# ethz-asl/object_keypoints

Hardware: AMD Instinct MI355X
Metric: frames/sec keypoint inference (511x511 -> heatmaps+3D) (higher is better)
Workload: dtype bf16

## Files before the change

### object_keypoints_amd/csrc/okp_fire2.hip

```cpp
#include <cstdio>
#include <cstring>

#include <cstdlib>

#include "okp_internal.h"

#ifdef OKP_F2_ABL_NOSTORE
#define F2_STORE(v, rs, off) do { if ((off) == 0x7ffffff0u) __builtin_amdgcn_raw_buffer_store_b128(v, rs, (int)(off), 0, 0); } while (0)
#else
#define F2_STORE(v, rs, off) __builtin_amdgcn_raw_buffer_store_b128(v, rs, (int)(off), 0, 0)
#endif


namespace {

constexpr uint32_t kInvalid = 0x80000000u;
typedef __attribute__((address_space(3))) void* lds_ptr_t;
typedef float f32x2 __attribute__((ext_vector_type(2)));

constexpr int SP = 128;
constexpr int PBI = 6;
constexpr int NST = 4;
constexpr int MAXIH = 6;
#ifndef OKP_F2_DIH
#define OKP_F2_DIH 5
#endif
constexpr int kDwmIH = OKP_F2_DIH;
static_assert(kDwmIH >= 1 && kDwmIH <= 5, "DWM tile: (rows + 2) x 18 squeeze pixels <= SP");
#ifdef OKP_F2_NO_REMAP
constexpr int XST = SP * 64;
#else
constexpr int XST = SP * 64 + 64;
#endif

template <int MID> struct FireLds {
  static constexpr int OFF_S = 0;
  static constexpr int OFF_X = OFF_S + SP * MID * 2;
  static constexpr int OFF_WD = OFF_X + NST * XST;
  static constexpr int OFF_TAB = OFF_WD + 10 * MID * 4;
  static constexpr int OFF_MASK = OFF_TAB + 2 * 96 * 4;
  static constexpr int BYTES = OFF_MASK + 16;
};

template <typename T>
__device__ __forceinline__ u32x4 relu_add_pack8(const f32x4& a0, const f32x4& a1, const u32x4& r) {
  u32x4 v;
#pragma unroll
  for (int b = 0; b < 2; ++b) {
    const f32x4& a = b ? a1 : a0;
#pragma unroll
    for (int h = 0; h < 2; ++h) {
      const f32x2 s2 = f32x2{a[2 * h], a[2 * h + 1]} + f32x2{H16<T>::lo(r[2 * b + h]), H16<T>::hi(r[2 * b + h])};
      v[2 * b + h] = okp_pack2<T>(s2[0], s2[1]);
    }
  }
  typedef short s16x8 __attribute__((ext_vector_type(8)));
  const s16x8 z = {0, 0, 0, 0, 0, 0, 0, 0};
  return __builtin_bit_cast(u32x4, __builtin_elementwise_max(__builtin_bit_cast(s16x8, v), z));
}

__device__ __forceinline__ int fastdiv(int x, const OkpFastDiv& f) {
  return f.mul ? (int)(__umulhi((uint32_t)x, f.mul) >> f.shift) : x;
}

__device__ __forceinline__ void wait_vm(int n) {
  switch (n) {
    case 0: asm volatile("s_waitcnt vmcnt(0)" ::: "memory"); break;
    case 1: asm volatile("s_waitcnt vmcnt(1)" ::: "memory"); break;
    case 2: asm volatile("s_waitcnt vmcnt(2)" ::: "memory"); break;
    case 3: asm volatile("s_waitcnt vmcnt(3)" ::: "memory"); break;
    case 4: asm volatile("s_waitcnt vmcnt(4)" ::: "memory"); break;
    case 5: asm volatile("s_waitcnt vmcnt(5)" ::: "memory"); break;
    case 6: asm volatile("s_waitcnt vmcnt(6)" ::: "memory"); break;
    case 7: asm volatile("s_waitcnt vmcnt(7)" ::: "memory"); break;
    default: asm volatile("s_waitcnt vmcnt(8)" ::: "memory"); break;
  }
}

#ifdef OKP_FIRE_STAMPS
#define F2_STAMP_ANY(i) do { if (lane == 0 && blockIdx.x < 16) { uint64_t t_; asm volatile("s_memtime %0\n s_waitcnt lgkmcnt(0)" : "=s"(t_) :: "memory"); p.dbg[(blockIdx.x * 8 + w) * 8 + (i)] = (uint32_t)t_; } } while (0)
#define F2_STAMP(i) do { if (second && lane == 0 && blockIdx.x < 16) { uint64_t t_; asm volatile("s_memtime %0\n s_waitcnt lgkmcnt(0)" : "=s"(t_) :: "memory"); p.dbg[(blockIdx.x * 8 + w) * 8 + (i)] = (uint32_t)t_; } } while (0)
#else
#define F2_STAMP(i) do {} while (0)
#define F2_STAMP_ANY(i) do {} while (0)
#endif

template <typename T, int CIN, int MID, int STR, bool DWM = false>
__global__ __launch_bounds__(MID * 2, MID == 128 ? 2 : 1) void okp_fire2_kernel(const OkpFire2Params p) {
  static_assert(STR == 1 || STR == 2, "stride of both branches");
  constexpr bool DWM2 = DWM && STR == 2;
  constexpr int D2H = 3, D2W = 8, D2SW = 2 * (D2W - 1) + 3, D2SH = 2 * (D2H - 1) + 3, D2B = 2;
  static_assert(D2SH * D2SW <= SP && D2B * 16 >= D2H * D2W + 8, "stride-2 matrix-pipe tile");
  constexpr int DIH = kDwmIH;
  constexpr int DSW = 18;
  constexpr int NSB = !DWM ? SP / 16 : STR == 1 ? ((DIH + 2) * DSW + 15) / 16 : (D2SH * D2SW + 15) / 16;
  constexpr int NW = MID / 32;
  constexpr int NT = 64 * NW;
  constexpr int HALF = MID;
  constexpr int KS1 = CIN / 32;
  constexpr int KS2 = MID / 32;
#ifdef OKP_F2_RESIDENT_W1
  constexpr bool RES = CIN <= 256;
  constexpr int DWB = 1;
#else
  constexpr bool RES = false;
#ifdef OKP_F2_RESIDENT_WA
  constexpr int DWB = (CIN == 256 && MID == 128) ? OKP_F2_RESIDENT_WA : 1;
#else
  constexpr int DWB = (CIN == 256 && MID == 128) ? 4 : 1;
#endif
#endif
#ifndef OKP_F2_RESWA
#define OKP_F2_RESWA 0
#endif
#ifdef OKP_F2_RESIDENT_WA
  constexpr bool RESWA = CIN == 256 && MID == 128;
#else
  constexpr bool RESWA = OKP_F2_RESWA && DWM && CIN == 256 && MID == 128;
#endif
  constexpr bool WRING = !RES && MID >= 192;
#ifndef OKP_F2_PIPE
#define OKP_F2_PIPE 0
#endif
  constexpr bool PIPE = OKP_F2_PIPE && DWM && CIN == 256 && MID == 128 && !RES && !WRING;
  constexpr int NWS = PIPE ? 4 : 3;
  constexpr int DW = !WRING ? 0 : MID == 192 ? 5 : 3;
  constexpr int SWM = ((MID / 8) % 16 == 0) ? 15 : 7;
  constexpr int CG = MID / 8;
  constexpr int NDM = (SP / 16 + NW - 1) / NW;
  constexpr bool RING_SKIP = STR == 1 && CIN == 2 * MID && KS1 / 2 <= NST;
  using L = FireLds<MID>;
  constexpr int OFF_S = L::OFF_S, OFF_X = L::OFF_X, OFF_WD = L::OFF_WD, OFF_TAB = L::OFF_TAB, OFF_MASK = L::OFF_MASK;
  constexpr int OFF_W1 = (L::BYTES + 1023) / 1024 * 1024;
  constexpr int LDS_TOTAL = WRING ? OFF_W1 + DW * NW * 2048 : L::BYTES;
  static_assert(NT / CG == 16 && LDS_TOTAL <= 160 * 1024, "thread mapping / LDS");
  __shared__ __attribute__((aligned(16))) char smem[LDS_TOTAL];
  const int tid = threadIdx.x;
  const int lane = tid & 63;
  const int w = __builtin_amdgcn_readfirstlane(tid >> 6);
  const int l16 = lane & 15, q = lane >> 4;

  const __amdgpu_buffer_rsrc_t rs_x = __builtin_amdgcn_make_buffer_rsrc(const_cast<void*>(p.x), 0, (int)p.x_bytes, 0x00020000);
  const __amdgpu_buffer_rsrc_t rs_o = __builtin_amdgcn_make_buffer_rsrc(p.out, 0, (int)p.out_bytes, 0x00020000);

  const int chq = 32 * w + 8 * q;
  const __amdgpu_buffer_rsrc_t rs_w1 = __builtin_amdgcn_make_buffer_rsrc(const_cast<void*>(p.w1), 0, NW * 2 * KS1 * 1024, 0x00020000);
  const uint32_t w1_voff = (uint32_t)lane * 16u;
  auto load_w1 = [&](int ks, u32x4 (&dst)[2]) {
#ifdef OKP_F2_ABL_NOWEIGHTS
    if (ks != 0) { dst[0] = u32x4{0x3c003c00u, 0u, 0u, 0u}; dst[1] = dst[0]; return; }
#endif
#pragma unroll
    for (int b = 0; b < 2; ++b)
      dst[b] = __builtin_amdgcn_raw_buffer_load_b128(rs_w1, (int)w1_voff, (int)(((uint32_t)(w * 2 + b) * KS1 + (uint32_t)ks) * 1024u), 0);
  };
  auto issue_w = [&](int ks) {
    if constexpr (WRING) {
#pragma unroll
      for (int b = 0; b < 2; ++b)
        __builtin_amdgcn_raw_ptr_buffer_load_lds(rs_w1, (lds_ptr_t)(smem + OFF_W1 + ((ks % DW) * NW + w) * 2048 + b * 1024), 16,
                                                 (int)(((uint32_t)(w * 2 + b) * KS1 + (uint32_t)ks) * 1024u + (uint32_t)lane * 16u), 0, 0, 0);
    }
  };
  auto first_weights = [&](u32x4 (&f)[RES ? KS1 : NWS][2]) {
    if constexpr (WRING) {
#pragma unroll
      for (int ks = 0; ks < DW; ++ks) issue_w(ks);
    } else if constexpr (!RES) {
      load_w1(0, f[0]); load_w1(1, f[1]);
    }
  };
  u32x4 w1f[RES ? KS1 : NWS][2];
  if constexpr (RES) {
#pragma unroll
    for (int ks = 0; ks < KS1; ++ks) load_w1(ks, w1f[ks]);
  }
  const u32x4* const wa_lane = static_cast<const u32x4*>(p.wa) + (size_t)w * 2 * KS2 * 64 + lane;
  u32x4 waf[2][KS2];
  if constexpr (RESWA) {
#pragma unroll
    for (int b = 0; b < 2; ++b)
#pragma unroll
      for (int ks = 0; ks < KS2; ++ks) waf[b][ks] = wa_lane[(size_t)(b * KS2 + ks) * 64];
  }
  const f32x4 b1v0 = *reinterpret_cast<const f32x4*>(p.b1 + chq), b1v1 = *reinterpret_cast<const f32x4*>(p.b1 + chq + 4);
  const f32x4 bav0 = *reinterpret_cast<const f32x4*>(p.ba + chq), bav1 = *reinterpret_cast<const f32x4*>(p.ba + chq + 4);
  uint32_t a_row[PBI], a_key[PBI];
#pragma unroll
  for (int pb = 0; pb < PBI; ++pb) {
    int ip = 16 * pb + l16;
    if (ip >= p.IP) ip = 0;
    const int iy = fastdiv(ip, p.div_iw), ix = ip - iy * p.IW;
    const int sp = (STR * iy + 1) * p.SW + STR * ix + 1;
    a_row[pb] = (uint32_t)sp * (MID * 2);
    a_key[pb] = (uint32_t)(sp & SWM);
  }
  const uint32_t xfrag_off = (uint32_t)l16 * 64u + (uint32_t)((q + 2 * (l16 >> 2)) & 3) * 16u;
  const uint32_t s_dst = (uint32_t)(OFF_S + l16 * (MID * 2) + (((4 * w + q) ^ (l16 & SWM)) << 4));
  constexpr bool UNI = (SP / 16) % NW == 0;
  const int nd = UNI ? NDM : (SP / 16 - w + NW - 1) / NW;
  int d_sy[NDM], d_sx[NDM];
  uint32_t d_chunk[NDM];
#pragma unroll
  for (int i = 0; i < NDM; ++i) {
    const int row = 16 * (w + NW * i) + (lane >> 2);
    d_sy[i] = fastdiv(row, p.div_sw);
    d_sx[i] = row - d_sy[i] * p.SW;
    if (row >= p.SH * p.SW) d_sy[i] = 1 << 20;
    d_chunk[i] = (uint32_t)(((lane & 3) - 2 * (row >> 2)) & 3) * 16u;
  }
  const int m_sy = tid < p.SH * p.SW ? fastdiv(tid, p.div_sw) : (1 << 20);
  const int m_sx = tid - fastdiv(tid, p.div_sw) * p.SW;

  auto tile_origin = [&](int slot, int& n, int& y0, int& x0) {
    const int xq = p.n_tiles >> 3, xr = p.n_tiles & 7, xcd = slot & 7;
    const int tile = (xcd < xr ? xcd * (xq + 1) : xr * (xq + 1) + (xcd - xr) * xq) + (slot >> 3);
    n = fastdiv(tile, p.div_tiles_frame);
    const int trem = tile - n * p.tiles_y * p.tiles_x;
    const int ty = fastdiv(trem, p.div_tiles_x);
    y0 = ty * p.IH;
    x0 = (trem - ty * p.tiles_x) * p.IW;
  };
  uint32_t d_off[NDM];
  auto tile_setup = [&](int tile) {
    int n, y0, x0;
    tile_origin(tile, n, y0, x0);
#pragma unroll
    for (int i = 0; i < NDM; ++i) {
      const int y = STR * y0 - 1 + d_sy[i], x = STR * x0 - 1 + d_sx[i];
// ... 535 lines not shown
          }
          } else {
#pragma unroll
          for (int sr = 0; sr < STR * (MAXIH - 1) + 3; ++sr) {
            if (sr < STR * (p.IH - 1) + 3) {
              const int sp = sr * p.SW + STR * ixc + dx;
              const u32x4 sv = *reinterpret_cast<const u32x4*>(smem + OFF_S + sp * (MID * 2) + ((cg ^ (sp & SWM)) << 4));
              f32x2 s2[4];
#pragma unroll
              for (int e = 0; e < 4; ++e) s2[e] = f32x2{H16<T>::lo(sv[e]), H16<T>::hi(sv[e])};
#pragma unroll
              for (int dy = 0; dy < 3; ++dy) {
                const int iy = (sr - dy) / STR;
                if (sr - dy >= 0 && (sr - dy) % STR == 0 && iy < MAXIH) {
#pragma unroll
                  for (int e = 0; e < 4; ++e) v[iy][e] = __builtin_elementwise_fma(s2[e], wt[dy][e], v[iy][e]);
                }
              }
            }
          }
          }
        }
#pragma unroll
        for (int iy = 0; iy < MAXIH; ++iy) {
          u32x4 o;
#pragma unroll
          for (int e = 0; e < 4; ++e) {
            const float lo = fmaxf(v[iy][e][0] + H16<T>::lo(rr[iy][e]), 0.f);
            const float hi = fmaxf(v[iy][e][1] + H16<T>::hi(rr[iy][e]), 0.f);
            o[e] = okp_pack2<T>(lo, hi);
          }
          F2_STORE(o, rs_o, oo[iy]);
        }
      }
    }
    F2_STAMP(4);
  }
  F2_STAMP_ANY(7);
}

}


bool okp_fire2_supported(int cin, int mid, int half, int stride) {
  if (half != mid) return false;
  if (stride == 1)
    return (cin == 256 && mid == 128) || (cin == 384 && mid == 192) || (cin == 512 && mid == 256) ||
           (cin == 384 && mid == 128) || (cin == 512 && mid == 192);
  return stride == 2 && ((cin == 256 && mid == 128) || (cin == 384 && mid == 192) || (cin == 384 && mid == 256) || (cin == 256 && mid == 192));
}

template <typename T>
static int launch_fire2_t(OkpFire2Params p, int cin, int mid, int stride, hipStream_t stream) {
  const long resident_wg = 256 * (mid == 128 ? 2 : 1);
  long best = -1;
  for (int ih = 1; ih <= p.Ho && ih <= MAXIH; ++ih)
    for (int iw = 1; iw <= p.Wo && iw <= 96; ++iw) {
      const int sh = stride * (ih - 1) + 3, sw = stride * (iw - 1) + 3;
      if (sh * sw > SP || ih * iw > 16 * PBI) continue;
      const long ty = (p.Ho + ih - 1) / ih, tx = (p.Wo + iw - 1) / iw;
      const long rounds = ((long)p.N * ty * tx + resident_wg - 1) / resident_wg;
      const long score = (rounds << 40) + (rounds == 1 ? (long)sh * sw + 8 * (16 - (iw < 16 ? iw : 16)) : ty * tx) * 4096 - iw;
      if (best < 0 || score < best) { best = score; p.IH = ih; p.IW = iw; p.SH = sh; p.SW = sw; p.tiles_y = (int)ty; p.tiles_x = (int)tx; }
    }
  if (stride == 2) {
    static const char* const e = getenv("OKP_F2_S2_TILE");
    int ih = 0, iw = 0;
    if (e && sscanf(e, "%d,%d", &ih, &iw) == 2 && ih >= 1 && ih <= MAXIH && iw >= 1 && (2 * (ih - 1) + 3) * (2 * (iw - 1) + 3) <= SP && ih * iw <= 16 * PBI) {
      p.IH = ih < p.Ho ? ih : p.Ho; p.IW = iw < p.Wo ? iw : p.Wo; p.SH = 2 * (p.IH - 1) + 3; p.SW = 2 * (p.IW - 1) + 3;
      p.tiles_y = (p.Ho + p.IH - 1) / p.IH; p.tiles_x = (p.Wo + p.IW - 1) / p.IW;
    }
  }
  static const bool dwm_on = [] { const char* e = getenv("OKP_F2_DWM"); return !(e && e[0] == '0'); }();
  static const int dwm_mid = [] { const char* e = getenv("OKP_F2_DWM_MID"); return e ? atoi(e) : 256; }();
  const bool dwm = dwm_on && stride == 1 && p.Wo % 16 == 0 && mid <= dwm_mid;
  if (dwm) {
    p.IH = p.Ho < kDwmIH ? p.Ho : kDwmIH; p.IW = 16; p.SH = p.IH + 2; p.SW = 18;
    p.tiles_y = (p.Ho + p.IH - 1) / p.IH; p.tiles_x = p.Wo / 16;
  }
  static const bool dwm2_on = [] { const char* e = getenv("OKP_F2_DWM_S2"); return !(e && e[0] == '0'); }();
  const bool dwm2 = dwm_on && dwm2_on && stride == 2 && p.Wo % 8 == 0 && mid <= dwm_mid;
  if (dwm2) {
    const long tx = p.Wo / 8;
    int ih = p.Ho < 3 ? p.Ho : 3;
    if (ih == 3 && (long)p.N * ((p.Ho + 1) / 2) * tx <= resident_wg) ih = 2;
    p.IH = ih; p.IW = 8; p.SH = 2 * (ih - 1) + 3; p.SW = 17;
    p.tiles_y = (p.Ho + ih - 1) / ih; p.tiles_x = (int)tx;
  }
  p.IP = p.IH * p.IW;
  p.RPR = (p.IW + 3) / 4;
  const long tiles = (long)p.N * p.tiles_y * p.tiles_x;
  if (tiles >= 0x7FFFFFFFl) { okp_set_error("okp_fire_forward: too many tiles"); return OKP_EINVAL; }
  p.n_tiles = (int)tiles;
  p.div_tiles_frame = okp_fastdiv((uint32_t)(p.tiles_y * p.tiles_x));
  p.div_tiles_x = okp_fastdiv((uint32_t)p.tiles_x);
  p.div_sw = okp_fastdiv((uint32_t)p.SW);
  p.div_iw = okp_fastdiv((uint32_t)p.IW);
  p.div_rpr = okp_fastdiv((uint32_t)p.RPR);
  const int resident = 256 * (mid == 128 ? 2 : 1);
  const dim3 grid((unsigned)(p.n_tiles < resident ? p.n_tiles : resident)), block((unsigned)(2 * mid));
#ifdef OKP_FIRE_STAMPS
  static uint32_t* dbg = nullptr;
  if (!dbg) (void)hipMalloc((void**)&dbg, 16 * 8 * 8 * 4);
  (void)hipMemsetAsync(dbg, 0, 16 * 8 * 8 * 4, stream);
  p.dbg = dbg;
  struct Print { OkpFire2Params p; int mid; hipStream_t stream; uint32_t* dbg; ~Print() {
    if (!getenv("OKP_FIRE_STAMPS_PRINT")) return;
    (void)hipStreamSynchronize(stream);
    uint32_t h[16 * 8 * 8];
    (void)hipMemcpy(h, dbg, sizeof(h), hipMemcpyDeviceToHost);
    const int nw = mid / 32;
    printf("fire2 stamps (tile %d x %d interior, %d tiles, %d waves): clocks per wave of the second tile: squeeze GEMM (ring) | s -> LDS + barrier | expand GEMM + stores | depth-wise branch (+ next tile's requests)\n", p.IH, p.IW, p.n_tiles, nw);
    double sum[4] = {0, 0, 0, 0}; int cnt = 0;
    for (int wg = 0; wg < 16; ++wg)
      for (int w = 0; w < nw; ++w) {
        const uint32_t* a = &h[(wg * 8 + w) * 8];
        if (!a[4]) continue;
        if (wg % 5 == 0 && (w == 0 || w == nw - 1)) printf("wg %2d wave %d: %6u | %6u | %6u | %6u\n", wg, w, a[1] - a[0], a[2] - a[1], a[3] - a[2], a[4] - a[3]);
        for (int i = 0; i < 4; ++i) sum[i] += a[i + 1] - a[i];
        ++cnt;
      }
    if (cnt) printf("mean: %.0f | %.0f | %.0f | %.0f  = %.0f clocks per tile\n", sum[0] / cnt, sum[1] / cnt, sum[2] / cnt, sum[3] / cnt, (sum[0] + sum[1] + sum[2] + sum[3]) / cnt);
    double pro = 0, all = 0; int c2 = 0;
    for (int wg = 0; wg < 16; ++wg)
      for (int w = 0; w < nw; ++w) { const uint32_t* a = &h[(wg * 8 + w) * 8]; if (!a[7]) continue; pro += a[6] - a[5]; all += a[7] - a[5]; ++c2; }
    if (c2) printf("whole kernel: prologue (first requests + constants -> LDS + barrier) %.0f clocks, entry to exit %.0f clocks\n", pro / c2, all / c2);
  } } print_at_exit{p, mid, stream, dbg};
#endif
  if (stride == 1) {
    if (dwm && cin == 256 && mid == 128) hipLaunchKernelGGL((okp_fire2_kernel<T, 256, 128, 1, true>), grid, block, 0, stream, p);
    else if (dwm && cin == 384 && mid == 192) hipLaunchKernelGGL((okp_fire2_kernel<T, 384, 192, 1, true>), grid, block, 0, stream, p);
    else if (dwm && cin == 512 && mid == 256) hipLaunchKernelGGL((okp_fire2_kernel<T, 512, 256, 1, true>), grid, block, 0, stream, p);
    else if (dwm && cin == 384 && mid == 128) hipLaunchKernelGGL((okp_fire2_kernel<T, 384, 128, 1, true>), grid, block, 0, stream, p);
    else if (dwm && cin == 512 && mid == 192) hipLaunchKernelGGL((okp_fire2_kernel<T, 512, 192, 1, true>), grid, block, 0, stream, p);
    else if (cin == 256 && mid == 128) hipLaunchKernelGGL((okp_fire2_kernel<T, 256, 128, 1>), grid, block, 0, stream, p);
    else if (cin == 384 && mid == 192) hipLaunchKernelGGL((okp_fire2_kernel<T, 384, 192, 1>), grid, block, 0, stream, p);
    else if (cin == 512 && mid == 256) hipLaunchKernelGGL((okp_fire2_kernel<T, 512, 256, 1>), grid, block, 0, stream, p);
    else if (cin == 384 && mid == 128) hipLaunchKernelGGL((okp_fire2_kernel<T, 384, 128, 1>), grid, block, 0, stream, p);
    else if (cin == 512 && mid == 192) hipLaunchKernelGGL((okp_fire2_kernel<T, 512, 192, 1>), grid, block, 0, stream, p);
    else { okp_set_error("okp_fire_forward: no streaming kernel for %d -> %d", cin, mid); return OKP_EINVAL; }
  } else if (dwm2 && cin == 256 && mid == 128) hipLaunchKernelGGL((okp_fire2_kernel<T, 256, 128, 2, true>), grid, block, 0, stream, p);
  else if (dwm2 && cin == 384 && mid == 192) hipLaunchKernelGGL((okp_fire2_kernel<T, 384, 192, 2, true>), grid, block, 0, stream, p);
  else if (dwm2 && cin == 384 && mid == 256) hipLaunchKernelGGL((okp_fire2_kernel<T, 384, 256, 2, true>), grid, block, 0, stream, p);
  else if (dwm2 && cin == 256 && mid == 192) hipLaunchKernelGGL((okp_fire2_kernel<T, 256, 192, 2, true>), grid, block, 0, stream, p);
  else if (cin == 256 && mid == 192) hipLaunchKernelGGL((okp_fire2_kernel<T, 256, 192, 2>), grid, block, 0, stream, p);
  else if (cin == 256 && mid == 128) hipLaunchKernelGGL((okp_fire2_kernel<T, 256, 128, 2>), grid, block, 0, stream, p);
  else if (cin == 384 && mid == 192) hipLaunchKernelGGL((okp_fire2_kernel<T, 384, 192, 2>), grid, block, 0, stream, p);
  else if (cin == 384 && mid == 256) hipLaunchKernelGGL((okp_fire2_kernel<T, 384, 256, 2>), grid, block, 0, stream, p);
  else { okp_set_error("okp_fire_forward: no streaming kernel for %d -> %d stride %d", cin, mid, stride); return OKP_EINVAL; }
  return okp_check_hip(hipGetLastError(), "okp_fire2 launch");
}

int okp_launch_fire2(int dtype, const OkpFire2Params& p, int cin, int mid, int stride, hipStream_t stream) {
  if (dtype == OKP_BF16) return launch_fire2_t<__bf16>(p, cin, mid, stride, stream);
  return launch_fire2_t<_Float16>(p, cin, mid, stride, stream);
}

extern "C" int okp_fire_forward(const okp_conv* squeeze, const okp_conv* expand, const float* dw_w_dev, const float* dw_bias_dev,
                                const okp_fire_args* a, void* stream) {
  if (!squeeze || !expand || !dw_w_dev || !dw_bias_dev || !a || !a->x.data || !a->out.data) { okp_set_error("okp_fire_forward: null argument"); return OKP_EINVAL; }
  const bool x3 = squeeze->dtype == OKP_F32X3;
  if (!(okp_is16(squeeze->dtype) || x3) || expand->dtype != squeeze->dtype) { okp_set_error("okp_fire_forward: the fused fire kernel takes bf16, fp16 or split-product (OKP_F32X3) plans of one type"); return OKP_EINVAL; }
  if (squeeze->n_taps != 1 || expand->n_taps != 1 || squeeze->n_src != 1 || expand->n_src != 1) { okp_set_error("okp_fire_forward: squeeze/expand must be single-tap 1x1 plans"); return OKP_EINVAL; }
  const int cin = squeeze->cin[0], mid = squeeze->cout, half = expand->cout;
  if (expand->cin[0] != mid || half != mid) { okp_set_error("okp_fire_forward: expects expand cin == squeeze cout == half (sr = 2)"); return OKP_EINVAL; }
  if (cin % 64 || mid % 64 || mid > 256) { okp_set_error("okp_fire_forward: cin %d / mid %d must be multiples of 64, mid <= 256", cin, mid); return OKP_EINVAL; }
  if (a->stride != 1 && a->stride != 2) { okp_set_error("okp_fire_forward: stride %d", a->stride); return OKP_EINVAL; }
  if (a->skip && (a->stride != 1 || cin != 2 * half)) { okp_set_error("okp_fire_forward: skip needs stride 1 and cin == cout"); return OKP_EINVAL; }
  const int ho = (a->x.h - 1) / a->stride + 1, wo = (a->x.w - 1) / a->stride + 1;
  if (a->out.h != ho || a->out.w != wo) { okp_set_error("okp_fire_forward: out is %dx%d, expected %dx%d", a->out.h, a->out.w, ho, wo); return OKP_EINVAL; }
  if (x3) {
    if (!okp_fire_x3_supported(cin, mid, half, a->stride, a->skip) || squeeze->n_single_slices || expand->n_single_slices || !squeeze->fragT_dev || !expand->fragT_dev) {
      okp_set_error("okp_fire_forward: the split-product one-launch kernel takes 256 -> 128 -> 256 at stride 1 with skip or at stride 2 without (three-term plans); run the squeeze plan and the fused tail instead");
      return OKP_EINVAL;
    }
    if (a->x.pix_stride % 4 || a->out.pix_stride % 4 || a->x.pix_stride < cin || a->out.pix_stride < 2 * half || ((uintptr_t)a->x.data) % 16 || ((uintptr_t)a->out.data) % 16) {
      okp_set_error("okp_fire_forward: views must be 16-byte aligned and wide enough"); return OKP_EINVAL;
    }
    if (a->x.bytes <= 0 || a->x.bytes >= 0x7FFF0000ll || a->out.bytes <= 0 || a->out.bytes >= 0x7FFF0000ll) { okp_set_error("okp_fire_forward: views must be < 2 GiB"); return OKP_EINVAL; }
    OkpFire2Params q;
    memset(&q, 0, sizeof(q));
    q.x = a->x.data; q.x_bytes = (uint32_t)a->x.bytes; q.H = a->x.h; q.W = a->x.w; q.x_ps = a->x.pix_stride;
    q.out = a->out.data; q.out_bytes = (uint32_t)a->out.bytes; q.Ho = ho; q.Wo = wo; q.out_ps = a->out.pix_stride;
    q.N = a->n; q.skip = a->skip;
    q.w1 = squeeze->fragT_dev; q.w1_cout_pad = squeeze->cout_pad; q.b1 = squeeze->bias_dev; q.s1 = squeeze->oscale_dev;
    q.wa = expand->fragT_dev; q.wa_cout_pad = expand->cout_pad; q.ba = expand->bias_dev; q.sa = expand->oscale_dev;
    q.wd = dw_w_dev; q.bd = dw_bias_dev; q.range_flag = squeeze->range_flag;
    return okp_launch_fire_x3(q, a->stride, (hipStream_t)stream);
  }
  if (a->x.pix_stride % 8 || a->out.pix_stride % 8 || a->x.pix_stride < cin || a->out.pix_stride < 2 * half ||
      ((uintptr_t)a->x.data) % 16 || ((uintptr_t)a->out.data) % 16) { okp_set_error("okp_fire_forward: views must be 16-byte aligned and wide enough"); return OKP_EINVAL; }
  if (a->x.bytes <= 0 || a->x.bytes >= 0x7FFF0000ll) { okp_set_error("okp_fire_forward: x spans %lld bytes; views must be < 2 GiB", (long long)a->x.bytes); return OKP_EINVAL; }
  if (!okp_fire2_supported(cin, mid, half, a->stride)) {
    okp_set_error("okp_fire_forward: no one-launch kernel for %d -> %d -> %d at stride %d; run the squeeze plan and the fused tail "
                  "(okp_conv_forward with dw_*) instead", cin, mid, 2 * half, a->stride);
    return OKP_EINVAL;
  }
  {
    if (a->out.bytes <= 0 || a->out.bytes >= 0x7FFF0000ll) { okp_set_error("okp_fire_forward: out spans %lld bytes; views must be < 2 GiB", (long long)a->out.bytes); return OKP_EINVAL; }
    OkpFire2Params q;
    memset(&q, 0, sizeof(q));
    q.x = a->x.data; q.x_bytes = (uint32_t)a->x.bytes; q.H = a->x.h; q.W = a->x.w; q.x_ps = a->x.pix_stride;
    q.out = a->out.data; q.out_bytes = (uint32_t)a->out.bytes; q.Ho = ho; q.Wo = wo; q.out_ps = a->out.pix_stride;
    q.N = a->n; q.skip = a->skip;
#if defined(OKP_FIRE_STAMPS) || defined(OKP_F2_ABL_NOSKIP)
    if (getenv("OKP_FIRE_NOSKIP")) q.skip = 0;
#endif
    if (int e = okp_ensure_frags(squeeze, (hipStream_t)stream)) return e;
    if (int e = okp_ensure_frags(expand, (hipStream_t)stream)) return e;
    q.w1 = squeeze->fragT_dev; q.w1_cout_pad = squeeze->cout_pad; q.b1 = squeeze->bias_dev;
    q.wa = expand->fragT_dev; q.wa_cout_pad = expand->cout_pad; q.ba = expand->bias_dev;
    q.wd = dw_w_dev; q.bd = dw_bias_dev;
    return okp_launch_fire2(squeeze->dtype, q, cin, mid, a->stride, (hipStream_t)stream);
  }
}
```

### object_keypoints_amd/csrc/okp_internal.h

```cpp
#pragma once
#include <hip/hip_runtime.h>
#include <stdint.h>
#include "okp.h"

#define OKP_MAX_TAPS 32

typedef float f32x4 __attribute__((ext_vector_type(4)));
typedef float f32x16 __attribute__((ext_vector_type(16)));
typedef __bf16 bf16x8 __attribute__((ext_vector_type(8)));
typedef __bf16 bf16x4 __attribute__((ext_vector_type(4)));
typedef __bf16 bf16x2 __attribute__((ext_vector_type(2)));
typedef _Float16 f16x8 __attribute__((ext_vector_type(8)));
typedef _Float16 f16x4 __attribute__((ext_vector_type(4)));
typedef _Float16 f16x2 __attribute__((ext_vector_type(2)));
typedef unsigned int u32x4 __attribute__((ext_vector_type(4)));
typedef unsigned int u32x2 __attribute__((ext_vector_type(2)));

template <typename T> struct H16;
template <> struct H16<__bf16> {
  using x2 = bf16x2; using x4 = bf16x4; using x8 = bf16x8;
  static constexpr int kDtype = OKP_BF16;
  static __device__ __forceinline__ f32x4 mfma16(const u32x4& a, const u32x4& b, const f32x4& c) {
#if defined(__HIP_DEVICE_COMPILE__)
    return __builtin_amdgcn_mfma_f32_16x16x32_bf16(__builtin_bit_cast(bf16x8, a), __builtin_bit_cast(bf16x8, b), c, 0, 0, 0);
#else
    return c;
#endif
  }
  static __device__ __forceinline__ f32x16 mfma32(const u32x4& a, const u32x4& b, const f32x16& c) {
#if defined(__HIP_DEVICE_COMPILE__)
    return __builtin_amdgcn_mfma_f32_32x32x16_bf16(__builtin_bit_cast(bf16x8, a), __builtin_bit_cast(bf16x8, b), c, 0, 0, 0);
#else
    return c;
#endif
  }
  static __device__ __forceinline__ float lo(uint32_t w) { return __builtin_bit_cast(float, w << 16); }
  static __device__ __forceinline__ float hi(uint32_t w) { return __builtin_bit_cast(float, w & 0xffff0000u); }
};
template <> struct H16<_Float16> {
  using x2 = f16x2; using x4 = f16x4; using x8 = f16x8;
  static constexpr int kDtype = OKP_F16;
  static __device__ __forceinline__ f32x4 mfma16(const u32x4& a, const u32x4& b, const f32x4& c) {
#if defined(__HIP_DEVICE_COMPILE__)
    return __builtin_amdgcn_mfma_f32_16x16x32_f16(__builtin_bit_cast(f16x8, a), __builtin_bit_cast(f16x8, b), c, 0, 0, 0);
#else
    return c;
#endif
  }
  static __device__ __forceinline__ f32x16 mfma32(const u32x4& a, const u32x4& b, const f32x16& c) {
#if defined(__HIP_DEVICE_COMPILE__)
    return __builtin_amdgcn_mfma_f32_32x32x16_f16(__builtin_bit_cast(f16x8, a), __builtin_bit_cast(f16x8, b), c, 0, 0, 0);
#else
    return c;
#endif
  }
  static __device__ __forceinline__ float lo(uint32_t w) { return (float)__builtin_bit_cast(f16x2, w)[0]; }
  static __device__ __forceinline__ float hi(uint32_t w) { return (float)__builtin_bit_cast(f16x2, w)[1]; }
};

static __device__ __forceinline__ void okp_split4(const f32x4& x, u32x2& hi, u32x2& lo) {
#if defined(__HIP_DEVICE_COMPILE__)
#pragma unroll
  for (int q = 0; q < 2; ++q) {
    const float xa = x[2 * q], xb = x[2 * q + 1];
    f16x2 h2; h2[0] = (_Float16)xa; h2[1] = (_Float16)xb;
    const uint32_t hw = __builtin_bit_cast(uint32_t, h2);
    float da, db;
    asm("v_fma_mix_f32 %0, %1, -1.0, %2 op_sel:[0,0,0] op_sel_hi:[1,0,0]" : "=v"(da) : "v"(hw), "v"(xa));
    asm("v_fma_mix_f32 %0, %1, -1.0, %2 op_sel:[1,0,0] op_sel_hi:[1,0,0]" : "=v"(db) : "v"(hw), "v"(xb));
    f16x2 l2; l2[0] = (_Float16)da; l2[1] = (_Float16)db;
    hi[q] = hw; lo[q] = __builtin_bit_cast(uint32_t, l2);
  }
#else
  hi = u32x2{0u, 0u}; lo = u32x2{0u, 0u};
#endif
}

#ifdef OKP_NO_RANGE_GUARD
static __device__ __forceinline__ bool okp_unsplittable(float) { return false; }
static __device__ __forceinline__ float okp_range_max(float m, float) { return m; }
#else
static __device__ __forceinline__ bool okp_unsplittable(float v) { return !(__builtin_fabsf(v) <= 65504.f); }
static __device__ __forceinline__ float okp_range_max(float m, float v) { return __builtin_fmaxf(m, __builtin_fabsf(v)); }
#endif
static __device__ __forceinline__ bool okp_range_exceeded(float m) { return !(m <= 65504.f); }
static __device__ __forceinline__ void okp_raise_range_flag(int32_t* flag, bool bad) {
#if defined(__HIP_DEVICE_COMPILE__)
  if (flag != nullptr && bad) atomicOr(flag, 1);
#endif
}

template <typename T> __device__ __forceinline__ uint32_t okp_pack2(float a, float b) {
  typedef float f32x2_ __attribute__((ext_vector_type(2)));
  return __builtin_bit_cast(uint32_t, __builtin_convertvector((f32x2_){a, b}, typename H16<T>::x2));
}
inline int okp_esz(int dtype) { return (dtype == OKP_F32 || dtype == OKP_F32X3) ? 4 : 2; }
inline bool okp_is16(int dtype) { return dtype == OKP_BF16 || dtype == OKP_F16; }

struct OkpSlice {
  uint8_t tap_lo, tap_hi, src, nvalid;
  int32_t c0_lo, c0_hi;
  int32_t pad;
};

struct OkpTapDev {
  int32_t dy, dx, src, pad;
};

struct OkpFastDiv {
  uint32_t mul, shift;
};
inline OkpFastDiv okp_fastdiv(uint32_t d) {
  OkpFastDiv f{0u, 0u};
  if (d <= 1) return f;
  uint32_t s = 0;
  while ((1ull << s) < d) ++s;
  f.mul = (uint32_t)((1ull << (31 + s)) / d + 1);
  f.shift = s - 1;
  return f;
}

struct OkpIgemmParams {
  const void* src[2];
  uint32_t src_bytes[2];
  int32_t srcH[2], srcW[2], src_pix_stride[2], conv_stride[2];
  const void* weights;
  uint32_t w_bytes;
  int32_t cout_pad;
  const float* bias;
  const float* oscale;
  const OkpSlice* slices;
  int32_t n_slices;
  int32_t n_taps;
  int32_t N, Ho, Wo;
  OkpFastDiv div_howo, div_wo;
  void* out;
  uint32_t out_bytes, res_bytes;
  int32_t OH, OW, out_step, out_oy, out_ox, out_pix_stride;
  int32_t cout;
  const void* res;
  int32_t res_pix_stride;
  int32_t act;
  int32_t n_co_tiles;
  const float* dw_w;
  const float* dw_bias;
  void* dw_out;
  const void* dw_res;
  int32_t dw_out_pix_stride, dw_res_pix_stride;
  int32_t n_tiles;
  int32_t n_classes, tiles_per_class, slices_per_class;
  int32_t n_single_slices;
  void* out16;
  int32_t out16_pix_stride, res16;
  int32_t src_pairs, out_pairs;
  int32_t out_sub2, OH2, OW2;
  int32_t mfma32;
  int32_t* range_flag;
  int64_t src_bytes64[2];
  OkpTapDev taps[OKP_MAX_TAPS];
};

struct OkpPatchStep {
  uint32_t tap_bytes;
  uint32_t nx_c0b;
  uint8_t pbuf, nx_k0, nx_k1, nx_geom;
  uint8_t geom, tx, c0q, grp_last;
};
#define OKP_PSTEP_CVT_SELF 2u
#define OKP_PSTEP_CVT_NEXT 4u
#define OKP_PATCH_MAX_GEOM 6
static_assert(OKP_PATCH_MAX_GEOM * 5 <= 32, "OkpPatchParams.geom_ph packs 5 bits per geometry into one u32");
struct OkpPatchGeom {
  const void* data; uint32_t bytes;
  int32_t H, W, pix_stride;
  int32_t PW, npx;
  int32_t oy, ox;
  int32_t step, conv_stride;
};
struct OkpPatchParams {
  OkpPatchGeom g[OKP_PATCH_MAX_GEOM];
  int32_t n_geom;
  uint32_t geom_ph, geom_src;
  const void* src_data[2]; uint32_t src_bytes[2];
  const void* weights; uint32_t w_bytes; int32_t cout_pad, cout;
  const float* bias;
  const float* oscale;
  const OkpPatchStep* steps; int32_t n_steps;
  int32_t N, H, W, tiles_y, tiles_x;
  int32_t n_classes, steps_per_class, tiles_per_class;
  int32_t OH, OW, out_step, out_oy, out_ox;
  OkpFastDiv div_tiles_frame, div_tiles_x;
  void* out; uint32_t out_bytes; int32_t out_pix_stride;
  const void* res; uint32_t res_bytes; int32_t res_pix_stride;
  int32_t act, n_co_tiles, n_tiles;
  uint32_t pairs;
  int32_t* range_flag;
  int64_t src_total_bytes[2];
  int64_t src_frame_bytes[2];
#ifdef OKP_PATCH_STAMPS
  uint32_t* dbg;
#endif
};

struct OkpFire2Params {
  const void* x; uint32_t x_bytes; int32_t H, W, x_ps;
  void* out; uint32_t out_bytes; int32_t Ho, Wo, out_ps;
  int32_t N, skip;
  const void* w1; int32_t w1_cout_pad; const float* b1;
  const void* wa; int32_t wa_cout_pad; const float* ba;
  const float* wd; const float* bd;
  const float* s1; const float* sa;
  int32_t* range_flag;
  int32_t SH, SW, IH, IW, IP, RPR, tiles_y, tiles_x, n_tiles;
  OkpFastDiv div_tiles_frame, div_tiles_x, div_sw, div_iw, div_rpr;
#ifdef OKP_FIRE_STAMPS
  uint32_t* dbg;
#endif
};

struct OkpFireChainModule {
  const void* w1; int32_t w1_cout_pad; const float* b1;
  const void* wa; int32_t wa_cout_pad; const float* ba;
  const float* wd; const float* bd;
};
struct OkpFireChainParams {
  const void* x; void* out; int32_t x_ps, out_ps, H, W, n_modules;
  int32_t He, We;
  OkpFireChainModule mod[OKP_FIRE_CHAIN_MAX];
#ifdef OKP_FIRE_STAMPS
  uint32_t* dbg;
#endif
};

struct okp_conv {
  int dtype;
  int n_src;
  int32_t cin[2];
  int32_t conv_stride[2];
  int32_t cout, cout_pad;
  int32_t n_taps;
  OkpTapDev taps[OKP_MAX_TAPS];
  int32_t n_slices;
  int32_t n_single_slices;
  int act;
  void* weights_dev;
  uint32_t w_bytes;
  float* bias_dev;
  float* oscale_dev;
  OkpSlice* slices_dev;
  OkpPatchStep* patch_steps_dev;
  int32_t patch_n_geom;
  int32_t patch_src[OKP_PATCH_MAX_GEOM], patch_PW[OKP_PATCH_MAX_GEOM], patch_PH[OKP_PATCH_MAX_GEOM], patch_oy[OKP_PATCH_MAX_GEOM], patch_ox[OKP_PATCH_MAX_GEOM], patch_step[OKP_PATCH_MAX_GEOM];
  void* frag_dev;
  int32_t* range_flag;
  void* fragT_dev;
};

void okp_set_error(const char* fmt, ...);
uint16_t okp_f32_to_16(int dtype, float f);
int okp_check_hip(hipError_t e, const char* what);

int okp_select_tile(int dtype, int cout_pad, long pixels);
int okp_launch_igemm(const okp_conv* plan, const OkpIgemmParams& p, int tile, hipStream_t stream);
int okp_ensure_frags(const okp_conv* plan, hipStream_t stream);
bool okp_fire2_supported(int cin, int mid, int half, int stride);
int okp_launch_fire2(int dtype, const OkpFire2Params& p, int cin, int mid, int stride, hipStream_t stream);
bool okp_fire_x3_supported(int cin, int mid, int half, int stride, int skip);
int okp_launch_fire_x3(OkpFire2Params p, int stride, hipStream_t stream);
bool okp_patch_supported(const okp_conv* plan, const OkpIgemmParams& p);
int okp_launch_igemm_patch(const okp_conv* plan, const OkpIgemmParams& p, hipStream_t stream);
int okp_fill_patch_params(const okp_conv* plan, const OkpIgemmParams& q, OkpPatchParams& p);
int okp_launch_igemm_patch_x3(const okp_conv* plan, const OkpPatchParams& p, hipStream_t stream);
```

Before: 13110.

## Add wide-tile fire kernel for small-grid 256->128 stride-1 fire layers

Adds a new specialized fused fire kernel (squeeze 1x1, expand 1x1 and depthwise 3x3 via matrix cores) with 8x32 output tiles, 512 threads, a persistent tile loop, and staged async buffer-to-LDS loads of both activations and weights. It is dispatched when cin=256, mid=128, stride 1 and the tile count fits in 256 blocks. The next tile's loads are prefetched during the current tile's epilogue. The aim is more reuse per halo and better occupancy of the small-grid layers, at the cost of a large LDS footprint and one block per CU.

```diff
diff --git a/object_keypoints_amd/csrc/okp_fire2.hip b/object_keypoints_amd/csrc/okp_fire2.hip
--- a/object_keypoints_amd/csrc/okp_fire2.hip
+++ b/object_keypoints_amd/csrc/okp_fire2.hip
@@ -42,39 +42,8 @@
   static constexpr int BYTES = OFF_MASK + 16;
 };
 
-template <typename T>
-__device__ __forceinline__ u32x4 relu_add_pack8(const f32x4& a0, const f32x4& a1, const u32x4& r) {
-  u32x4 v;
-#pragma unroll
-  for (int b = 0; b < 2; ++b) {
-    const f32x4& a = b ? a1 : a0;
-#pragma unroll
-    for (int h = 0; h < 2; ++h) {
-      const f32x2 s2 = f32x2{a[2 * h], a[2 * h + 1]} + f32x2{H16<T>::lo(r[2 * b + h]), H16<T>::hi(r[2 * b + h])};
-      v[2 * b + h] = okp_pack2<T>(s2[0], s2[1]);
-    }
-  }
-  typedef short s16x8 __attribute__((ext_vector_type(8)));
-  const s16x8 z = {0, 0, 0, 0, 0, 0, 0, 0};
-  return __builtin_bit_cast(u32x4, __builtin_elementwise_max(__builtin_bit_cast(s16x8, v), z));
-}
-
 __device__ __forceinline__ int fastdiv(int x, const OkpFastDiv& f) {
   return f.mul ? (int)(__umulhi((uint32_t)x, f.mul) >> f.shift) : x;
-}
-
-__device__ __forceinline__ void wait_vm(int n) {
-  switch (n) {
-    case 0: asm volatile("s_waitcnt vmcnt(0)" ::: "memory"); break;
-    case 1: asm volatile("s_waitcnt vmcnt(1)" ::: "memory"); break;
-    case 2: asm volatile("s_waitcnt vmcnt(2)" ::: "memory"); break;
-    case 3: asm volatile("s_waitcnt vmcnt(3)" ::: "memory"); break;
-    case 4: asm volatile("s_waitcnt vmcnt(4)" ::: "memory"); break;
-    case 5: asm volatile("s_waitcnt vmcnt(5)" ::: "memory"); break;
-    case 6: asm volatile("s_waitcnt vmcnt(6)" ::: "memory"); break;
-    case 7: asm volatile("s_waitcnt vmcnt(7)" ::: "memory"); break;
-    default: asm volatile("s_waitcnt vmcnt(8)" ::: "memory"); break;
-  }
 }
 
 #ifdef OKP_FIRE_STAMPS
@@ -916,6 +885,7 @@
 }
 
 int okp_launch_fire2(int dtype, const OkpFire2Params& p, int cin, int mid, int stride, hipStream_t stream) {
+  if (okp_fire4_applies(p.N, cin, mid, stride, p.Ho, p.Wo)) return okp_launch_fire4(dtype, p, stream);
   if (dtype == OKP_BF16) return launch_fire2_t<__bf16>(p, cin, mid, stride, stream);
   return launch_fire2_t<_Float16>(p, cin, mid, stride, stream);
 }
diff --git a/object_keypoints_amd/csrc/okp_fire4.hip b/object_keypoints_amd/csrc/okp_fire4.hip
--- /dev/null
+++ b/object_keypoints_amd/csrc/okp_fire4.hip
@@ -0,0 +1,333 @@
+#include "okp_internal.h"
+
+namespace {
+
+typedef __attribute__((address_space(3))) void* lds_ptr_t;
+constexpr uint32_t kInvalid = 0x80000000u;
+
+constexpr int MID = 128, CIN = 256;
+constexpr int KS1 = CIN / 32, KS2 = MID / 32;
+constexpr int TIH = 8, TIW = 32;
+constexpr int TSW = TIW + 2, TSH = TIH + 2;
+constexpr int NSQ = TSH * TSW;
+constexpr int NSB = (NSQ + 15) / 16;
+constexpr int HB = NSB / 2;
+constexpr int NST = 4, NPRE = 2;
+constexpr int DW = 3;
+constexpr int XST = NSB * 1024;
+constexpr int NDM = (NSB + 7) / 8;
+constexpr int OFF_S = NPRE * XST;
+constexpr int OFF_W1 = OFF_S + NSQ * MID * 2;
+constexpr int OFF_WD = OFF_W1 + DW * 8192;
+constexpr int OFF_MASK = OFF_WD + 10 * MID * 4;
+constexpr int LDS_BYTES = OFF_MASK + 12 * 4;
+static_assert(NSB % 2 == 0 && NST * XST <= OFF_W1 && LDS_BYTES <= 160 * 1024, "LDS layout");
+
+struct VmTab { int one[KS1], x[KS1]; };
+constexpr VmTab make_vm_tab() {
+  VmTab t{};
+  int kind[64] = {}, idx[64] = {}, step[64] = {}, ne = 0;
+  for (int s = 0; s < DW; ++s) { kind[ne] = 0; idx[ne] = s; step[ne] = -1; ++ne; }
+  for (int s = 0; s < NPRE; ++s) { kind[ne] = 1; idx[ne] = s; step[ne] = -1; ++ne; }
+  for (int s = NPRE; s < NST; ++s) { kind[ne] = 1; idx[ne] = s; step[ne] = 0; ++ne; }
+  for (int j = 1; j < KS1; ++j) {
+    if (j - 1 + DW < KS1) { kind[ne] = 0; idx[ne] = j - 1 + DW; step[ne] = j; ++ne; }
+    if (j + NST - 1 < KS1) { kind[ne] = 1; idx[ne] = j + NST - 1; step[ne] = j; ++ne; }
+  }
+  for (int ks = 1; ks < KS1; ++ks) {
+    int last = -1;
+    for (int e = 0; e < ne; ++e) if (idx[e] == ks) last = e;
+    for (int e = last + 1; e < ne; ++e)
+      if (step[e] < ks) { if (kind[e]) ++t.x[ks]; else ++t.one[ks]; }
+  }
+  return t;
+}
+constexpr VmTab kVm = make_vm_tab();
+static_assert(kVm.one[1] == 0 && kVm.x[1] == 2 && kVm.one[3] == 1 && kVm.x[3] == 2 && kVm.one[7] == 0 && kVm.x[7] == 0, "wait counts");
+static_assert(kVm.one[2] + kVm.x[2] * NDM <= 8 && kVm.one[5] + kVm.x[5] * NDM <= 8, "wait_vm takes counts up to 8");
+
+__device__ __forceinline__ int fastdiv4(int x, const OkpFastDiv& f) {
+  return f.mul ? (int)(__umulhi((uint32_t)x, f.mul) >> f.shift) : x;
+}
+
+template <typename T>
+__global__ __launch_bounds__(512, 1) void okp_fire4_kernel(const OkpFire2Params p) {
+  __shared__ __attribute__((aligned(16))) char smem[LDS_BYTES];
+  const int tid = threadIdx.x;
+  const int lane = tid & 63;
+  const int w = __builtin_amdgcn_readfirstlane(tid >> 6);
+  const int v = w & 3, h = w >> 2;
+  const int l16 = lane & 15, q = lane >> 4;
+  const int chq = 32 * v + 8 * q;
+
+  const __amdgpu_buffer_rsrc_t rs_x = __builtin_amdgcn_make_buffer_rsrc(const_cast<void*>(p.x), 0, (int)p.x_bytes, 0x00020000);
+  const __amdgpu_buffer_rsrc_t rs_o = __builtin_amdgcn_make_buffer_rsrc(p.out, 0, (int)p.out_bytes, 0x00020000);
+  const __amdgpu_buffer_rsrc_t rs_w1 = __builtin_amdgcn_make_buffer_rsrc(const_cast<void*>(p.w1), 0, 4 * 2 * KS1 * 1024, 0x00020000);
+  auto issue_w = [&](int ks) {
+    __builtin_amdgcn_raw_ptr_buffer_load_lds(rs_w1, (lds_ptr_t)(smem + OFF_W1 + (ks % DW) * 8192 + w * 1024), 16,
+                                             (int)(((uint32_t)w * KS1 + (uint32_t)ks) * 1024u + (uint32_t)lane * 16u), 0, 0, 0);
+  };
+
+  const int nd = w < NSB - 16 ? 3 : 2;
+  int d_sy[NDM], d_sx[NDM];
+  uint32_t d_chunk[NDM];
+#pragma unroll
+  for (int i = 0; i < NDM; ++i) {
+    const int row = 16 * (w + 8 * i) + (lane >> 2);
+    d_sy[i] = row < NSQ ? row / TSW : (1 << 20);
+    d_sx[i] = row % TSW;
+    d_chunk[i] = (uint32_t)(((lane & 3) - 2 * (row >> 2)) & 3) * 16u;
+  }
+  const int m_sy = tid < NSQ ? tid / TSW : (1 << 20), m_sx = tid % TSW;
+
+  auto tile_origin = [&](int slot, int& n, int& y0, int& x0) {
+    const int xq = p.n_tiles >> 3, xr = p.n_tiles & 7, xcd = slot & 7;
+    const int tile = (xcd < xr ? xcd * (xq + 1) : xr * (xq + 1) + (xcd - xr) * xq) + (slot >> 3);
+    n = fastdiv4(tile, p.div_tiles_frame);
+    const int trem = tile - n * p.tiles_y * p.tiles_x;
+    const int ty = fastdiv4(trem, p.div_tiles_x);
+    y0 = ty * TIH;
+    x0 = (trem - ty * p.tiles_x) * TIW;
+  };
+  uint32_t d_off[NDM];
+  auto tile_setup = [&](int tile) {
+    int n, y0, x0;
+    tile_origin(tile, n, y0, x0);
+#pragma unroll
+    for (int i = 0; i < NDM; ++i) {
+      const int y = y0 - 1 + d_sy[i], x = x0 - 1 + d_sx[i];
+      const bool ok = y >= 0 && y < p.H && x >= 0 && x < p.W;
+      d_off[i] = ok ? (uint32_t)(((long)n * p.H + y) * p.W + x) * (uint32_t)(p.x_ps * 2) + d_chunk[i] : kInvalid;
+    }
+    if (w < NSB * 16 / 64 + 1) {
+      const int y = y0 - 1 + m_sy, x = x0 - 1 + m_sx;
+      const unsigned long long m = __ballot(y >= 0 && y < p.H && x >= 0 && x < p.W);
+      if (lane == 0) {
+        uint32_t* mk = reinterpret_cast<uint32_t*>(smem + OFF_MASK);
+        mk[2 * w] = (uint32_t)m;
+        mk[2 * w + 1] = (uint32_t)(m >> 32);
+      }
+    }
+  };
+  auto issue_x = [&](int ks, int stage) {
+#pragma unroll
+    for (int i = 0; i < NDM; ++i)
+      if (i < nd)
+        __builtin_amdgcn_raw_ptr_buffer_load_lds(rs_x, (lds_ptr_t)(smem + stage * XST + (w + 8 * i) * 1024), 16,
+                                                 (int)(d_off[i] == kInvalid ? kInvalid : d_off[i] + (uint32_t)ks * 64u), 0, 0, 0);
+  };
+
+  int tile = blockIdx.x;
+  if (tile >= p.n_tiles) return;
+  tile_setup(tile);
+#pragma unroll
+  for (int s = 0; s < DW; ++s) issue_w(s);
+#pragma unroll
+  for (int s = 0; s < NPRE; ++s) issue_x(s, s);
+  const u32x4* const wa_lane = static_cast<const u32x4*>(p.wa) + (size_t)v * 2 * KS2 * 64 + lane;
+  const f32x4 b1v0 = *reinterpret_cast<const f32x4*>(p.b1 + chq), b1v1 = *reinterpret_cast<const f32x4*>(p.b1 + chq + 4);
+  const f32x4 bav0 = *reinterpret_cast<const f32x4*>(p.ba + chq), bav1 = *reinterpret_cast<const f32x4*>(p.ba + chq + 4);
+  {
+    float cv[3];
+#pragma unroll
+    for (int k = 0; k < 3; ++k) {
+      const int i = tid + k * 512;
+      cv[k] = i < 9 * MID ? p.wd[i] : i < 10 * MID ? p.bd[i - 9 * MID] : 0.f;
+    }
+#pragma unroll
+    for (int k = 0; k < 3; ++k) {
+      const int i = tid + k * 512;
+      const uint32_t wq = (i & 1) ? okp_pack2<T>(0.f, cv[k]) : okp_pack2<T>(cv[k], 0.f);
+      if (i < 10 * MID) reinterpret_cast<uint32_t*>(smem + OFF_WD)[i] = i < 9 * MID ? wq : __builtin_bit_cast(uint32_t, cv[k]);
+    }
+  }
+  __syncthreads();
+
+  const uint32_t xfrag = (uint32_t)(HB * h) * 1024u + (uint32_t)l16 * 64u + (uint32_t)((q + 2 * (l16 >> 2)) & 3) * 16u;
+  const uint32_t wfrag = (uint32_t)OFF_W1 + (uint32_t)(2 * v) * 1024u + (uint32_t)lane * 16u;
+
+  for (; tile < p.n_tiles; tile += gridDim.x) {
+    int n, y0, x0;
+    tile_origin(tile, n, y0, x0);
+    int qt = q, l16t = l16;
+    asm volatile("" : "+v"(qt), "+v"(l16t));
+
+    f32x4 acc[HB][2];
+#pragma unroll
+    for (int j = 0; j < HB; ++j) { acc[j][0] = b1v0; acc[j][1] = b1v1; }
+#pragma unroll
+    for (int ks = 0; ks < KS1; ++ks) {
+      if (ks == 0) wait_vm(0);
+      else wait_vm(kVm.one[ks] + kVm.x[ks] * nd);
+      asm volatile("s_waitcnt lgkmcnt(0)" ::: "memory");
+      __builtin_amdgcn_s_barrier();
+      if (ks == 0) {
+#pragma unroll
+        for (int s = NPRE; s < NST; ++s) issue_x(s, s);
+      } else {
+        if (ks - 1 + DW < KS1) issue_w(ks - 1 + DW);
+        if (ks + NST - 1 < KS1) issue_x(ks + NST - 1, (ks + NST - 1) % NST);
+      }
+      const char* st = smem + (ks % NST) * XST + xfrag;
+      u32x4 a[HB], wr[2];
+#pragma unroll
+      for (int b = 0; b < 2; ++b) wr[b] = *reinterpret_cast<const u32x4*>(smem + wfrag + (ks % DW) * 8192 + b * 1024);
+#pragma unroll
+      for (int j = 0; j < HB; ++j) a[j] = *reinterpret_cast<const u32x4*>(st + j * 1024);
+#pragma unroll
+      for (int j = 0; j < HB; ++j)
+#pragma unroll
+        for (int b = 0; b < 2; ++b) acc[j][b] = H16<T>::mfma16(wr[b], a[j], acc[j][b]);
+    }
+    u32x4 waf[2][KS2];
+#pragma unroll
+    for (int b = 0; b < 2; ++b)
+#pragma unroll
+      for (int ks = 0; ks < KS2; ++ks) waf[b][ks] = wa_lane[(size_t)(b * KS2 + ks) * 64];
+    asm volatile("s_waitcnt lgkmcnt(0)" ::: "memory");
+    __builtin_amdgcn_s_barrier();
+    {
+      const uint32_t* mk = reinterpret_cast<const uint32_t*>(smem + OFF_MASK);
+#pragma unroll
+      for (int j = 0; j < HB; ++j) {
+        const int pb = HB * h + j;
+        const int row = 16 * pb + l16t;
+        const bool ok = (mk[pb >> 1] >> (16 * (pb & 1) + l16t)) & 1u;
+        u32x4 o;
+#pragma unroll
+        for (int b = 0; b < 2; ++b) {
+          const uint32_t p0 = okp_pack2<T>(acc[j][b][0], acc[j][b][1]), p1 = okp_pack2<T>(acc[j][b][2], acc[j][b][3]);
+          o[2 * b] = ok ? p0 : 0u;
+          o[2 * b + 1] = ok ? p1 : 0u;
+        }
+        if (j < HB - 1 || row < NSQ)
+          *reinterpret_cast<u32x4*>(smem + OFF_S + row * (MID * 2) + (((4 * v + qt) ^ (row & 15)) << 4)) = o;
+      }
+    }
+    __syncthreads();
+
+    const uint32_t pix0 = (uint32_t)(((long)n * p.Ho + y0) * p.Wo + x0 + 16 * h);
+    const uint32_t lane_x = (uint32_t)l16t * (uint32_t)(p.x_ps * 2) + (uint32_t)chq * 2u, lane_o = (uint32_t)l16t * (uint32_t)(p.out_ps * 2) + (uint32_t)chq * 2u;
+    const uint32_t rowx = (uint32_t)(p.W * p.x_ps * 2), rowo = (uint32_t)(p.Wo * p.out_ps * 2), noskip = p.skip ? 0u : kInvalid;
+    uint32_t o_off[TIH], x_off[TIH];
+    {
+      uint32_t sx = pix0 * (uint32_t)(p.x_ps * 2), so = pix0 * (uint32_t)(p.out_ps * 2);
+#pragma unroll
+      for (int iy = 0; iy < TIH; ++iy) {
+        const uint32_t bad = y0 + iy < p.Ho ? 0u : kInvalid;
+        o_off[iy] = lane_o + (so | bad);
+        x_off[iy] = lane_x + (sx | bad | noskip);
+        sx += rowx;
+        so += rowo;
+      }
+    }
+    {
+      u32x4 rsk[TIH];
+#pragma unroll
+      for (int iy = 0; iy < TIH; ++iy) rsk[iy] = __builtin_amdgcn_raw_buffer_load_b128(rs_x, (int)x_off[iy], 0, 0);
+      f32x4 ac2[TIH][2];
+#pragma unroll
+      for (int iy = 0; iy < TIH; ++iy) { ac2[iy][0] = bav0; ac2[iy][1] = bav1; }
+      const uint32_t srow = (uint32_t)(TSW + 1 + 16 * h) + (uint32_t)l16t;
+#pragma unroll
+      for (int ks = 0; ks < KS2; ++ks) {
+        u32x4 a[TIH];
+#pragma unroll
+        for (int iy = 0; iy < TIH; ++iy) {
+          const uint32_t row = srow + (uint32_t)(iy * TSW);
+          a[iy] = *reinterpret_cast<const u32x4*>(smem + OFF_S + row * (MID * 2) + ((((uint32_t)(4 * ks) + (uint32_t)qt) ^ (row & 15u)) << 4));
+        }
+#pragma unroll
+        for (int iy = 0; iy < TIH; ++iy)
+#pragma unroll
+          for (int b = 0; b < 2; ++b) ac2[iy][b] = H16<T>::mfma16(waf[b][ks], a[iy], ac2[iy][b]);
+      }
+#pragma unroll
+      for (int iy = 0; iy < TIH; ++iy)
+        __builtin_amdgcn_raw_buffer_store_b128(relu_add_pack8<T>(ac2[iy][0], ac2[iy][1], rsk[iy]), rs_o, (int)o_off[iy], 0, 0);
+    }
+    asm volatile("" ::: "memory");
+
+    u32x4 rr2[TIH];
+#pragma unroll
+    for (int iy = 0; iy < TIH; ++iy) rr2[iy] = __builtin_amdgcn_raw_buffer_load_b128(rs_x, (int)(x_off[iy] + (uint32_t)(MID * 2)), 0, 0);
+    {
+      const int next = tile + gridDim.x;
+      if (next < p.n_tiles) {
+        tile_setup(next);
+#pragma unroll
+        for (int s = 0; s < DW; ++s) issue_w(s);
+#pragma unroll
+        for (int s = 0; s < NPRE; ++s) issue_x(s, s);
+      }
+    }
+    const float* const bl = reinterpret_cast<const float*>(smem + OFF_WD) + 9 * MID + chq;
+    const f32x4 bdv0 = *reinterpret_cast<const f32x4*>(bl), bdv1 = *reinterpret_cast<const f32x4*>(bl + 4);
+    const uint32_t am = (qt == (l16t >> 2)) ? 0xffffffffu : 0u;
+    const uint32_t m_lo = (l16t & 2) ? 0u : am, m_hi = (l16t & 2) ? am : 0u;
+    const uint32_t wt_lane = (uint32_t)OFF_WD + (uint32_t)(chq + (l16t & 3)) * 4u;
+    const uint32_t cx = (uint32_t)(4 * v) + (uint32_t)qt;
+#pragma unroll
+    for (int g = 0; g < 2; ++g) {
+      constexpr int GR = TIH / 2;
+      f32x4 acd[GR][2];
+#pragma unroll
+      for (int iy = 0; iy < GR; ++iy) { acd[iy][0] = bdv0; acd[iy][1] = bdv1; }
+      u32x4 a0[3], a1[3];
+#pragma unroll
+      for (int dy = 0; dy < 3; ++dy) { a0[dy] = u32x4{0u, 0u, 0u, 0u}; a1[dy] = u32x4{0u, 0u, 0u, 0u}; }
+#pragma unroll
+      for (int dx = 0; dx < 3; ++dx) {
+#pragma unroll
+        for (int dy = 0; dy < 3; ++dy) {
+          const uint32_t v0 = *reinterpret_cast<const uint32_t*>(smem + wt_lane + ((dy * 3 + dx) * MID) * 4);
+          const uint32_t v1 = *reinterpret_cast<const uint32_t*>(smem + wt_lane + ((dy * 3 + dx) * MID + 4) * 4);
+          a0[dy][0] = v0 & m_lo; a0[dy][1] = v0 & m_hi;
+          a1[dy][2] = v1 & m_lo; a1[dy][3] = v1 & m_hi;
+        }
+        u32x4 bf[GR + 2];
+#pragma unroll
+        for (int r = 0; r < GR + 2; ++r) {
+          const uint32_t sp = (uint32_t)((GR * g + r) * TSW + dx + 16 * h) + (uint32_t)l16t;
+          bf[r] = *reinterpret_cast<const u32x4*>(smem + OFF_S + sp * (MID * 2) + ((cx ^ (sp & 15u)) << 4));
+        }
+#pragma unroll
+        for (int r = 0; r < GR + 2; ++r)
+#pragma unroll
+          for (int dy = 0; dy < 3; ++dy) {
+            const int iy = r - dy;
+            if (iy >= 0 && iy < GR) {
+              acd[iy][0] = H16<T>::mfma16(a0[dy], bf[r], acd[iy][0]);
+              acd[iy][1] = H16<T>::mfma16(a1[dy], bf[r], acd[iy][1]);
+            }
+          }
+      }
+#pragma unroll
+      for (int iy = 0; iy < GR; ++iy)
+        __builtin_amdgcn_raw_buffer_store_b128(relu_add_pack8<T>(acd[iy][0], acd[iy][1], rr2[GR * g + iy]), rs_o, (int)(o_off[GR * g + iy] + (uint32_t)(MID * 2)), 0, 0);
+    }
+  }
+}
+
+}
+
+bool okp_fire4_applies(int n, int cin, int mid, int stride, int ho, int wo) {
+  static const bool on = [] { const char* e = getenv("OKP_F2_WIDE"); return !(e && e[0] == '0'); }();
+  if (!(on && cin == CIN && mid == MID && stride == 1 && wo % TIW == 0 && ho >= TIH)) return false;
+  return (long)n * ((ho + TIH - 1) / TIH) * (wo / TIW) <= 256;
+}
+
+int okp_launch_fire4(int dtype, OkpFire2Params p, hipStream_t stream) {
+  p.IH = TIH; p.IW = TIW; p.SH = TSH; p.SW = TSW; p.IP = TIH * TIW; p.RPR = 0;
+  p.tiles_y = (p.Ho + TIH - 1) / TIH;
+  p.tiles_x = p.Wo / TIW;
+  const long tiles = (long)p.N * p.tiles_y * p.tiles_x;
+  if (tiles >= 0x7FFFFFFFl) { okp_set_error("okp_fire_forward: too many tiles"); return OKP_EINVAL; }
+  p.n_tiles = (int)tiles;
+  p.div_tiles_frame = okp_fastdiv((uint32_t)(p.tiles_y * p.tiles_x));
+  p.div_tiles_x = okp_fastdiv((uint32_t)p.tiles_x);
+  const dim3 grid((unsigned)(p.n_tiles < 256 ? p.n_tiles : 256)), block(512);
+  if (dtype == OKP_BF16) hipLaunchKernelGGL((okp_fire4_kernel<__bf16>), grid, block, 0, stream, p);
+  else hipLaunchKernelGGL((okp_fire4_kernel<_Float16>), grid, block, 0, stream, p);
+  return okp_check_hip(hipGetLastError(), "okp_fire4 launch");
+}
diff --git a/object_keypoints_amd/csrc/okp_internal.h b/object_keypoints_amd/csrc/okp_internal.h
--- a/object_keypoints_amd/csrc/okp_internal.h
+++ b/object_keypoints_amd/csrc/okp_internal.h
@@ -94,6 +94,38 @@
   typedef float f32x2_ __attribute__((ext_vector_type(2)));
   return __builtin_bit_cast(uint32_t, __builtin_convertvector((f32x2_){a, b}, typename H16<T>::x2));
 }
+template <typename T>
+static __device__ __forceinline__ u32x4 relu_add_pack8(const f32x4& a0, const f32x4& a1, const u32x4& r) {
+  typedef float f32x2 __attribute__((ext_vector_type(2)));
+  u32x4 v;
+#pragma unroll
+  for (int b = 0; b < 2; ++b) {
+    const f32x4& a = b ? a1 : a0;
+#pragma unroll
+    for (int h = 0; h < 2; ++h) {
+      const f32x2 s2 = f32x2{a[2 * h], a[2 * h + 1]} + f32x2{H16<T>::lo(r[2 * b + h]), H16<T>::hi(r[2 * b + h])};
+      v[2 * b + h] = okp_pack2<T>(s2[0], s2[1]);
+    }
+  }
+  typedef short s16x8 __attribute__((ext_vector_type(8)));
+  const s16x8 z = {0, 0, 0, 0, 0, 0, 0, 0};
+  return __builtin_bit_cast(u32x4, __builtin_elementwise_max(__builtin_bit_cast(s16x8, v), z));
+}
+
+static __device__ __forceinline__ void wait_vm(int n) {
+  switch (n) {
+    case 0: asm volatile("s_waitcnt vmcnt(0)" ::: "memory"); break;
+    case 1: asm volatile("s_waitcnt vmcnt(1)" ::: "memory"); break;
+    case 2: asm volatile("s_waitcnt vmcnt(2)" ::: "memory"); break;
+    case 3: asm volatile("s_waitcnt vmcnt(3)" ::: "memory"); break;
+    case 4: asm volatile("s_waitcnt vmcnt(4)" ::: "memory"); break;
+    case 5: asm volatile("s_waitcnt vmcnt(5)" ::: "memory"); break;
+    case 6: asm volatile("s_waitcnt vmcnt(6)" ::: "memory"); break;
+    case 7: asm volatile("s_waitcnt vmcnt(7)" ::: "memory"); break;
+    default: asm volatile("s_waitcnt vmcnt(8)" ::: "memory"); break;
+  }
+}
+
 inline int okp_esz(int dtype) { return (dtype == OKP_F32 || dtype == OKP_F32X3) ? 4 : 2; }
 inline bool okp_is16(int dtype) { return dtype == OKP_BF16 || dtype == OKP_F16; }
 
@@ -265,6 +297,8 @@
 int okp_ensure_frags(const okp_conv* plan, hipStream_t stream);
 bool okp_fire2_supported(int cin, int mid, int half, int stride);
 int okp_launch_fire2(int dtype, const OkpFire2Params& p, int cin, int mid, int stride, hipStream_t stream);
+bool okp_fire4_applies(int n, int cin, int mid, int stride, int ho, int wo);
+int okp_launch_fire4(int dtype, OkpFire2Params p, hipStream_t stream);
 bool okp_fire_x3_supported(int cin, int mid, int half, int stride, int skip);
 int okp_launch_fire_x3(OkpFire2Params p, int stride, hipStream_t stream);
 bool okp_patch_supported(const okp_conv* plan, const OkpIgemmParams& p);
```

Result: no change. 12990 (median of 6 runs) (-0.9%).
